# yu45020/Text_Segmentation_Image_Inpainting

Hardware: NVIDIA H100
Metric: PartialConv UNet 512x512 images/sec (fwd+bwd) (higher is better)
Workload: dtype bf16

## Files before the change

### text_segmentation_image_inpainting_b200/csrc/conv_stem.cu

```cuda
#include <string.h>

#include <algorithm>

#include "pcb_common.cuh"

namespace {

constexpr int S2D_C = 32;
constexpr int SK = 4;

size_t rup256(size_t v) { return (v + 255) / 256 * 256; }
size_t s2d_bytes(const pcb_conv *c) { return rup256(static_cast<size_t>(c->n) * (c->h / 2) * (c->w / 2) * S2D_C * sizeof(bf16)); }
size_t dwsub_bytes(const pcb_conv *c) { return rup256(sizeof(float) * c->cout * SK * SK * S2D_C); }

}

StemPlan pcb_stem_plan(const pcb_conv *c) {
    StemPlan K;
    memset(&K, 0, sizeof(K));
    if (c->dtype != PCB_BF16 || c->groups != 1 || c->nparts != 1 || c->kh != 7 || c->kw != 7 || c->stride != 2 || c->pad_h != 3 || c->pad_w != 3 ||
        c->dil != 1) return K;
    const pcb_part &p = c->parts[0];
    if (p.x_up || p.c > 8 || p.x_cstride != 8 || (p.mask && p.mask_up != 0) || ((c->h | c->w) & 1)) return K;
    if (p.x && (reinterpret_cast<uintptr_t>(p.x) & 15)) return K;
    if (c->ho != c->h / 2 || c->wo != c->w / 2 || c->cout < 32 || (c->cout & 7)) return K;
    pcb_conv &S = K.sub;
    S.n = c->n; S.h = c->h / 2; S.w = c->w / 2; S.cin = S2D_C; S.cout = c->cout; S.kh = S.kw = SK; S.stride = 1; S.pad_h = S.pad_w = 2; S.dil = 1;
    S.groups = 1; S.ho = S.h; S.wo = S.w; S.dtype = PCB_BF16; S.no_guard = c->no_guard; S.nparts = 1;
    S.parts[0].x = nullptr; S.parts[0].mask = nullptr; S.parts[0].c = S2D_C; S.parts[0].x_cstride = S2D_C;
    if (!pcb_tc_eligible(&S)) return K;
    size_t de;
    pcb_tc_weight_layout(&S, &K.sub_fe, &de);
    K.sub_fe = (K.sub_fe + 63) / 64 * 64;
    K.fwd_extra = K.sub_fe + 2 * static_cast<size_t>(c->cout) * SK * SK * S2D_C;
    K.workspace = s2d_bytes(c) + dwsub_bytes(c) + pcb_tc_workspace(&S);
    K.ok = true;
    return K;
// ... 8 lines not shown
        const int a = static_cast<int>(i & 1);
        const long long cell = i >> 1;
        const int sx = static_cast<int>(cell % ws);
        const long long t = cell / ws;
        const int sy = static_cast<int>(t % hs), img = static_cast<int>(t / hs);
        const long long q = (static_cast<long long>(img) * h + 2 * sy + a) * w + 2 * sx;
        uint4 v0 = __ldg(reinterpret_cast<const uint4 *>(x + q * 8)), v1 = __ldg(reinterpret_cast<const uint4 *>(x + q * 8 + 8));
        if (mask) {
            if (mask[q] == 0) v0 = make_uint4(0u, 0u, 0u, 0u);
            if (mask[q + 1] == 0) v1 = make_uint4(0u, 0u, 0u, 0u);
        }
        uint4 *dst = reinterpret_cast<uint4 *>(xs + cell * S2D_C + a * 16);
        dst[0] = v0; dst[1] = v1;
    }
}

__global__ void stem_weight_kernel(const float *__restrict__ w, float *__restrict__ wsub, int cout, int cin) {
    const int i = blockIdx.x * blockDim.x + threadIdx.x;
    if (i >= cout * SK * SK * S2D_C) return;
    const int k = i % S2D_C, jb = (i / S2D_C) % SK, ja = (i / (S2D_C * SK)) % SK, co = i / (S2D_C * SK * SK);
    const int ch = k & 7, b = (k >> 3) & 1, a = k >> 4;
    const int ty = 2 * ja + a - 1, tx = 2 * jb + b - 1;
    wsub[i] = (ty >= 0 && ty < 7 && tx >= 0 && tx < 7 && ch < cin) ? w[((static_cast<long long>(co) * 7 + ty) * 7 + tx) * cin + ch] : 0.f;
}

__global__ void stem_dw_gather_kernel(const float *__restrict__ dwsub, float *__restrict__ dw, int cout, int cin) {
    const int i = blockIdx.x * blockDim.x + threadIdx.x;
    if (i >= cout * 49 * cin) return;
    const int ch = i % cin, tx = (i / cin) % 7, ty = (i / (cin * 7)) % 7, co = i / (cin * 49);
    const int ja = (ty + 1) >> 1, a = (ty + 1) & 1, jb = (tx + 1) >> 1, b = (tx + 1) & 1;
    dw[i] += dwsub[((static_cast<long long>(co) * SK + ja) * SK + jb) * S2D_C + (a * 2 + b) * 8 + ch];
}

int run_s2d(const pcb_conv *c, bf16 *xs, cudaStream_t st) {
    const pcb_part &p = c->parts[0];
    PCB_CHECK(p.x != nullptr, "space-to-depth stem: null x");
    const long long total = static_cast<long long>(c->n) * (c->h / 2) * (c->w / 2) * 2;
    const int grid = static_cast<int>(std::max<long long>(1, std::min<long long>((total + 255) / 256, 16ll * pcb_num_sms())));
    s2d_kernel<<<grid, 256, 0, st>>>(static_cast<const bf16 *>(p.x), p.mask, xs, c->n, c->h, c->w);
    PCB_LAUNCH_CHECK();
    return 0;
}

}

int pcb_stem_weight_prepare(const pcb_conv *c, const StemPlan &K, const float *w_master, void *w_fwd_extra, bool zero_padding, cudaStream_t st) {
    PCB_CHECK(K.ok && w_fwd_extra, "space-to-depth stem: weight prepare on a layer that does not take this path");
    float *wsub = reinterpret_cast<float *>(static_cast<bf16 *>(w_fwd_extra) + K.sub_fe);
    const int total = c->cout * SK * SK * S2D_C;
    stem_weight_kernel<<<(total + 255) / 256, 256, 0, st>>>(w_master, wsub, c->cout, c->cin);
    PCB_LAUNCH_CHECK();
    return pcb_tc_weight_prepare(&K.sub, wsub, w_fwd_extra, nullptr, zero_padding, st);
}

int pcb_stem_forward(const pcb_conv *c, const StemPlan &K, const void *w_fwd_extra, const float *bias, void *y, int y_cstride,
                     const float *msum, void *workspace, double *bn_sums, const pcb_ep *ep, cudaStream_t st) {
    PCB_CHECK(K.ok && workspace, "space-to-depth stem forward: wrong layer / no workspace");
    uint8_t *ws = static_cast<uint8_t *>(workspace);
    bf16 *xs = reinterpret_cast<bf16 *>(ws);
    if (int rc = run_s2d(c, xs, st)) return rc;
    pcb_conv sub = K.sub;
    sub.parts[0].x = xs;
    uint64_t *sub_ws = reinterpret_cast<uint64_t *>(ws + s2d_bytes(c) + dwsub_bytes(c));
    if (int rc = pcb_tc_forward_mask_pass(&sub, sub_ws, st)) return rc;
    return pcb_tc_forward_ws(&sub, w_fwd_extra, bias, y, y_cstride, msum, sub_ws, true, bn_sums, ep, st);
}

int pcb_stem_wgrad(const pcb_conv *c, const StemPlan &K, const void *dc, int dc_cstride, float *dw, void *workspace, bool zero_dw,
                   cudaStream_t st) {
    PCB_CHECK(K.ok && workspace, "space-to-depth stem wgrad: wrong layer / no workspace");
    if (zero_dw) PCB_CUDA(cudaMemsetAsync(dw, 0, sizeof(float) * c->cout * 49 * c->cin, st));
    uint8_t *ws = static_cast<uint8_t *>(workspace);
    bf16 *xs = reinterpret_cast<bf16 *>(ws);
    float *dwsub = reinterpret_cast<float *>(ws + s2d_bytes(c));
    void *sub_ws = ws + s2d_bytes(c) + dwsub_bytes(c);
    if (int rc = run_s2d(c, xs, st)) return rc;
    pcb_conv sub = K.sub;
    sub.parts[0].x = xs;
    if (int rc = pcb_tc_wgrad(&sub, dc, dc_cstride, dwsub, sub_ws, true, st)) return rc;
    const int total = c->cout * 49 * c->cin;
    stem_dw_gather_kernel<<<(total + 255) / 256, 256, 0, st>>>(dwsub, dw, c->cout, c->cin);
    PCB_LAUNCH_CHECK();
    return 0;
}
```

### text_segmentation_image_inpainting_b200/csrc/conv_tc.cu

```cuda
#include <cuda.h>
#include <stdlib.h>
#include <string.h>

#include <algorithm>

#include "pcb_common.cuh"
#include "pcb_ptx.cuh"

namespace {

constexpr int BLOCK_M = 128;
constexpr int BLOCK_K = 64;
constexpr int A_STAGE_BYTES = BLOCK_M * 128;
constexpr int NUM_PRODUCER_THREADS = 128;
constexpr int TC_MAX_PARTS = 2;
constexpr int MMA_WARPS = 8;
constexpr int MMA_THREADS = MMA_WARPS * 32;
constexpr int acc_pitch(int block_n) { return block_n + 4; }
constexpr int acc_stage_bytes(int block_n) { return BLOCK_M * acc_pitch(block_n) * 4; }

inline int rup(int v, int m) { return (v + m - 1) / m * m; }

struct TcPart {
    const bf16 *x;
// ... 1781 lines not shown
#pragma unroll
        for (int i = 0; i < 4; ++i) {
            const int ci = ci0 + ty + 8 * i;
            if (co < P.cout && ci < P.cin) {
                int p = 0;
                while (p + 1 < P.nparts && ci >= P.choff[p] + P.c[p]) ++p;
                const int kpos = P.koff[p] + (ci - P.choff[p]);
                w_dg[static_cast<long long>(kpos) * P.kd + static_cast<long long>(tap) * P.cout64 + co] = __float2bfloat16_rn(tile[tx][ty + 8 * i]);
            }
        }
    }
}

__global__ void tc_weight_prepare_kernel(const float *__restrict__ wm, const WPrepParams P, bf16 *__restrict__ w_fwd, bf16 *__restrict__ w_dg) {
    const long long total = static_cast<long long>(P.cout) * P.taps * P.cin;
    for (long long i = blockIdx.x * static_cast<long long>(blockDim.x) + threadIdx.x; i < total; i += static_cast<long long>(gridDim.x) * blockDim.x) {
        const int ci = static_cast<int>(i % P.cin);
        const long long t = i / P.cin;
        const int tap = static_cast<int>(t % P.taps), co = static_cast<int>(t / P.taps);
        const bf16 v = __float2bfloat16_rn(wm[i]);
        if (P.rowpack) {
            const int tr = tap / P.kw, tc = tap - tr * P.kw;
            w_fwd[static_cast<long long>(co) * P.kf + tr * 64 + tc * 8 + ci] = v;
        } else {
            int p = 0;
            while (p + 1 < P.nparts && ci >= P.choff[p] + P.c[p]) ++p;
            const int kpos = P.koff[p] + (ci - P.choff[p]);
            w_fwd[static_cast<long long>(co) * P.kf + static_cast<long long>(tap) * P.ktap + kpos] = v;
            if (w_dg) w_dg[static_cast<long long>(kpos) * P.kd + static_cast<long long>(tap) * P.cout64 + co] = v;
        }
    }
}

typedef CUresult (*EncodeTiledFn)(CUtensorMap *, CUtensorMapDataType, cuuint32_t, void *, const cuuint64_t *,
                                  const cuuint64_t *, const cuuint32_t *, const cuuint32_t *, CUtensorMapInterleave,
                                  CUtensorMapSwizzle, CUtensorMapL2promotion, CUtensorMapFloatOOBfill);

EncodeTiledFn get_encode_fn() {
    static EncodeTiledFn fn = nullptr;
    if (!fn) {
        void *p = nullptr;
        cudaDriverEntryPointQueryResult qres;
        if (cudaGetDriverEntryPoint("cuTensorMapEncodeTiled", &p, cudaEnableDefault, &qres) == cudaSuccess &&
            qres == cudaDriverEntryPointSuccess)
            fn = reinterpret_cast<EncodeTiledFn>(p);
    }
    return fn;
}

int make_tmap_2d(CUtensorMap *tm, const void *base, long long rows, long long cols, long long pitch_elems, int box_rows) {
    EncodeTiledFn enc = get_encode_fn();
    PCB_CHECK(enc != nullptr, "cuTensorMapEncodeTiled not available from the driver");
    cuuint64_t dims[2] = {static_cast<cuuint64_t>(cols), static_cast<cuuint64_t>(rows)};
    cuuint64_t strides[1] = {static_cast<cuuint64_t>(pitch_elems) * 2};
    cuuint32_t box[2] = {64, static_cast<cuuint32_t>(box_rows)};
    cuuint32_t estr[2] = {1, 1};
    CUresult r = enc(tm, CU_TENSOR_MAP_DATA_TYPE_BFLOAT16, 2, const_cast<void *>(base), dims, strides, box, estr,
                     CU_TENSOR_MAP_INTERLEAVE_NONE, CU_TENSOR_MAP_SWIZZLE_128B, CU_TENSOR_MAP_L2_PROMOTION_L2_256B,
                     CU_TENSOR_MAP_FLOAT_OOB_FILL_NONE);
    PCB_CHECK(r == CUDA_SUCCESS, "cuTensorMapEncodeTiled failed (%d) rows=%lld cols=%lld pitch=%lld box_rows=%d base=%p", (int)r,
              rows, cols, pitch_elems, box_rows, base);
    return 0;
}

int make_tmap_nhwc(CUtensorMap *tm, const void *base, int channels, int w, int h, int n, long long cstride, int bx, int by, int bn, int es) {
    EncodeTiledFn enc = get_encode_fn();
    PCB_CHECK(enc != nullptr, "cuTensorMapEncodeTiled not available from the driver");
    cuuint64_t dims[4] = {static_cast<cuuint64_t>(channels), static_cast<cuuint64_t>(w), static_cast<cuuint64_t>(h), static_cast<cuuint64_t>(n)};
    cuuint64_t strides[3] = {static_cast<cuuint64_t>(cstride) * 2, static_cast<cuuint64_t>(w) * cstride * 2, static_cast<cuuint64_t>(h) * w * cstride * 2};
    cuuint32_t box[4] = {64, static_cast<cuuint32_t>(bx * es), static_cast<cuuint32_t>(by * es), static_cast<cuuint32_t>(bn)};
    cuuint32_t estr[4] = {1, static_cast<cuuint32_t>(es), static_cast<cuuint32_t>(es), 1};
    CUresult r = enc(tm, CU_TENSOR_MAP_DATA_TYPE_BFLOAT16, 4, const_cast<void *>(base), dims, strides, box, estr,
                     CU_TENSOR_MAP_INTERLEAVE_NONE, CU_TENSOR_MAP_SWIZZLE_128B, CU_TENSOR_MAP_L2_PROMOTION_L2_256B,
                     CU_TENSOR_MAP_FLOAT_OOB_FILL_NONE);
    PCB_CHECK(r == CUDA_SUCCESS, "cuTensorMapEncodeTiled(4D) failed (%d) c=%d w=%d h=%d n=%d cstride=%lld box=%d,%d,%d es=%d base=%p", (int)r,
              channels, w, h, n, cstride, bx, by, bn, es, base);
    return 0;
}

int *abort_flag_ptr() {
    static int *flag[PCB_MAX_DEVICES] = {};
    const int dev = pcb_cur_device();
    if (!flag[dev]) {
        if (cudaMalloc(&flag[dev], sizeof(int)) != cudaSuccess) { flag[dev] = nullptr; return nullptr; }
        cudaMemset(flag[dev], 0, sizeof(int));
    }
    return flag[dev];
}

bool is_rowpack(const pcb_conv *c) { return c->nparts == 1 && c->cin <= 8 && c->kw <= 8 && c->parts[0].x_up == 0; }

bool common_ok(const pcb_conv *c) {
    if (c->dtype != PCB_BF16 || c->groups != 1 || c->kh * c->kw > 64) return false;
    if (c->stride & (c->stride - 1)) return false;
    const long long lim = (1ll << 31) - 1;
    if (static_cast<long long>(c->n) * c->ho * c->wo * rup(c->cout, 64) > lim) return false;
    if (c->nparts < 1 || c->nparts > TC_MAX_PARTS) return false;
    for (int p = 0; p < c->nparts; ++p) {
        const pcb_part &pt = c->parts[p];
        if (pt.x_cstride % 8 != 0 || pt.x_cstride < rup(pt.c, 8)) return false;
        if (static_cast<long long>(c->n) * (c->h >> pt.x_up) * (c->w >> pt.x_up) * pt.x_cstride > lim) return false;
        if (pt.x && (reinterpret_cast<uintptr_t>(pt.x) & 15)) return false;
    }
    if (is_rowpack(c)) return c->cout >= 16;
    return c->cin >= 32 || c->cout >= 32;
}

struct Layout {
    int rowpack, ktap, cout64, rows_f, bn_f;
    long long kf, kd;
    int koff[TC_MAX_PARTS], kext[TC_MAX_PARTS];
};

Layout layout_of(const pcb_conv *c) {
    Layout L;
    memset(&L, 0, sizeof(L));
    L.rowpack = is_rowpack(c);
    const int taps = c->kh * c->kw;
    if (L.rowpack) {
        L.ktap = 64; L.koff[0] = 0; L.kext[0] = 64;
        L.kf = static_cast<long long>(c->kh) * 64;
// ... 605 lines not shown
    const DirPlan &F = T.fwd;
    PCB_CHECK(T.m_out < (1ll << 31), "problem too large");
    PCB_CHECK(y_cstride % 8 == 0 && y_cstride >= c->cout, "tensor-core forward: y channel stride must be a multiple of 8 and >= cout");
    PCB_CHECK(bn_sums == nullptr || T.fuses_epilogue, "fused BatchNorm statistics requested from a kernel that does not produce them");
    PCB_CHECK(ep == nullptr || T.fuses_epilogue, "fused BatchNorm + activation requested from a kernel that does not apply it");
    if (!mask_pass_done && T.fwd_tapmask)
        if (int rc = launch_tapmask(c, tapmask, st)) return rc;
    const bf16 *wf = static_cast<const bf16 *>(w_fwd);
    if (F.route == ROUTE_STEM) return pcb_stem_forward(c, T.stem, wf + T.extra_fwd_off, bias, y, y_cstride, msum, tapmask, bn_sums, ep, st);
    if (F.route == ROUTE_K2R) return pcb_k2r_forward(c, T.k2r, smallco_layout(L), w_fwd, wf + T.extra_fwd_off, bias, y, y_cstride, msum, tapmask, st);
    if (F.route == ROUTE_SMALLCO) return pcb_smallco_forward(c, smallco_layout(L), w_fwd, bias, y, y_cstride, msum, st);
    TcParams P;
    base_params(P, c, L);
    P.m_total = static_cast<int>(T.m_out);
    fill_parts(c, L, P.parts, tapmask, T.m_out);
    P.bias = bias; P.msum = msum; P.y = static_cast<bf16 *>(y); P.y_cstride = y_cstride; P.abort_flag = flag;
    P.bn_sums = bn_sums; P.bn_c = c->cout;
    set_ep(P, ep);
    P.ncols = L.rows_f;
    CUtensorMap tm;
    if (int rc = make_tmap_2d(&tm, w_fwd, L.rows_f, L.kf, L.kf, F.bn)) return rc;
    if (F.route == ROUTE_TMA) {
        P.box_w = F.box_w; P.box_h = F.box_h; P.box_n = F.box_n;
        CUtensorMap ta[TC_MAX_PARTS];
        if (int rc = a_operand_maps(c, T, tapmask, F.box_w + (F.halo ? (c->kw - 1) * c->dil : 0), F.box_h, F.box_n, ta, &P.use_fix, st)) return rc;
        P.ncols = (c->cout <= 32) ? 32 : L.rows_f;
        P.wk_base = 0; P.wk_col = L.ktap; P.wk_row = c->kw * L.ktap;
        return launch_tma<0>(P, tm, ta[0], ta[1], F.bn, F.halo, st);
    }
    P.hg = F.hg;
    return launch_tc<0>(P, tm, F.bn, st);
}

bool pcb_tc_dgrad_fuses_relu(const pcb_conv *c) { return tc_plan(c).dg_fuses_relu; }

int pcb_tc_dgrad(const pcb_conv *c, const void *dc, int dc_cstride, const void *w_dgrad, void *const *dx, const int *dx_cstride,
                 cudaStream_t st, const void *relu_x, int relu_cstride) {
    const TcPlan T = tc_plan(c);
    const Layout &L = T.L;
    const DirPlan &D = T.dg;
    PCB_CHECK(D.route != ROUTE_NONE, "data gradient of a row-packed (cin <= 8) tensor-core layer: set force_generic and pass KRSC weights");
    PCB_CHECK(w_dgrad != nullptr && (reinterpret_cast<uintptr_t>(dc) & 15) == 0, "pcb_pconv_backward_data: w_dgrad required / dc misaligned");
    PCB_CHECK(relu_x == nullptr || (T.dg_fuses_relu && relu_cstride % 8 == 0 && relu_cstride >= rup(c->cin, 8) &&
                                    (reinterpret_cast<uintptr_t>(relu_x) & 15) == 0),
              "tensor-core dgrad: the ReLU backward is fused only on the TMA-fed stride-1 kernel (16-byte aligned input, channel stride %% 8 == 0)");
    int *flag = abort_flag_ptr();
    PCB_CHECK(flag != nullptr, "cudaMalloc(abort flag) failed");
    PCB_CHECK(T.m_in < (1ll << 31), "problem too large");
    PCB_CHECK(dc_cstride % 8 == 0 && dc_cstride >= rup(c->cout, 8), "tensor-core dgrad: dc channel stride must be a multiple of 8");
    const bf16 *wd = static_cast<const bf16 *>(w_dgrad);
    if (D.route == ROUTE_K2R) return pcb_k2r_dgrad(c, T.k2r, smallco_layout(L), dc, dc_cstride, w_dgrad, wd + T.extra_dg_off, dx, dx_cstride, st);
    if (D.route == ROUTE_SMALLCO) return pcb_smallco_dgrad(c, smallco_layout(L), dc, dc_cstride, w_dgrad, dx, dx_cstride, st);
    const SpPlan &SPL = T.sp;
    void *dx_local[TC_MAX_PARTS] = {nullptr, nullptr};
    for (int p = 0; p < c->nparts && p < TC_MAX_PARTS; ++p) dx_local[p] = dx[p];
    if (SPL.ok) {
        if (dx[SPL.pu] != nullptr)
            if (int rc = sp_dgrad_up(c, SPL, L, dc, dc_cstride, wd + T.sp_off, dx[SPL.pu], dx_cstride[SPL.pu], flag, st)) return rc;
        dx_local[SPL.pu] = nullptr;
        if (SPL.ps < 0 || dx[SPL.ps] == nullptr) return 0;
    }
    dx = dx_local;
    TcParams P;
    base_params(P, c, L);
    P.m_total = static_cast<int>(T.m_in);
    fill_parts(c, L, P.parts, nullptr, 0);
// ... 148 lines not shown
```

### text_segmentation_image_inpainting_b200/csrc/pcb_common.cuh

```cuda
#pragma once
#include <cuda_bf16.h>
#include <cuda_runtime.h>
#include <stdint.h>
#include <stdio.h>

#include "../../include/pconv_b200.h"

int pcb_set_error(const char *fmt, ...);
void pcb_count_launch(int n = 1);

#define PCB_CHECK(cond, ...)                       \
    do {                                           \
        if (!(cond)) return pcb_set_error(__VA_ARGS__); \
    } while (0)

#define PCB_CUDA(expr)                                                                           \
    do {                                                                                         \
        cudaError_t _e = (expr);                                                                 \
        if (_e != cudaSuccess)                                                                   \
            return pcb_set_error("%s:%d: %s -> %s", __FILE__, __LINE__, #expr, cudaGetErrorString(_e)); \
    } while (0)

#define PCB_LAUNCH_CHECK()                                                                        \
    do {                                                                                         \
        cudaError_t _e = cudaGetLastError();                                                     \
        if (_e != cudaSuccess)                                                                   \
            return pcb_set_error("%s:%d: kernel launch -> %s", __FILE__, __LINE__, cudaGetErrorString(_e)); \
        pcb_count_launch();                                                                      \
    } while (0)

constexpr int PCB_MAX_DEVICES = 64;

static inline int pcb_cur_device() {
// ... 69 lines not shown
    }
};
template <> struct Vec8<float> {
    static __device__ __forceinline__ void load(const float *p, float (&v)[8]) {
        float4 a = reinterpret_cast<const float4 *>(p)[0], b = reinterpret_cast<const float4 *>(p)[1];
        v[0] = a.x; v[1] = a.y; v[2] = a.z; v[3] = a.w; v[4] = b.x; v[5] = b.y; v[6] = b.z; v[7] = b.w;
    }
    static __device__ __forceinline__ void store(float *p, const float (&v)[8]) {
        reinterpret_cast<float4 *>(p)[0] = make_float4(v[0], v[1], v[2], v[3]);
        reinterpret_cast<float4 *>(p)[1] = make_float4(v[4], v[5], v[6], v[7]);
    }
};

__device__ __forceinline__ float warp_sum(float v) {
#pragma unroll
    for (int o = 16; o > 0; o >>= 1) v += __shfl_xor_sync(0xffffffffu, v, o);
    return v;
}

struct pcb_ep { const float *scale, *shift; int act; float slope; };

int pcb_generic_forward(const pcb_conv *c, const void *w, const float *bias, void *y, int y_cstride, const float *msum, cudaStream_t st);
int pcb_generic_dgrad(const pcb_conv *c, const void *dc, int dc_cstride, const void *w_krsc, void *const *dx, const int *dx_cstride,
                      cudaStream_t st);
int pcb_generic_wgrad(const pcb_conv *c, const void *dc, int dc_cstride, float *dw, bool zero_dw, cudaStream_t st);
int pcb_mask_sums(const pcb_conv *c, float *msum, uint8_t *newmask, cudaStream_t st);
bool pcb_tc_eligible(const pcb_conv *c);
size_t pcb_tc_workspace(const pcb_conv *c);
void pcb_tc_weight_layout(const pcb_conv *c, size_t *fwd_elems, size_t *dgrad_elems);
int pcb_tc_weight_prepare(const pcb_conv *c, const float *w_master, void *w_fwd, void *w_dgrad, bool zero_padding, cudaStream_t st);
int pcb_tc_forward_mask_pass(const pcb_conv *c, uint64_t *tapmask, cudaStream_t st);
int pcb_tc_forward_ws(const pcb_conv *c, const void *w_fwd, const float *bias, void *y, int y_cstride, const float *msum,
                      uint64_t *tapmask, bool mask_pass_done, double *bn_sums, const pcb_ep *ep, cudaStream_t st);
bool pcb_tc_fuses_epilogue(const pcb_conv *c);
bool pcb_tc_subpixel(const pcb_conv *c);
int pcb_tc_dgrad(const pcb_conv *c, const void *dc, int dc_cstride, const void *w_dgrad, void *const *dx, const int *dx_cstride,
                 cudaStream_t st, const void *relu_x = nullptr, int relu_cstride = 0);
bool pcb_tc_dgrad_fuses_relu(const pcb_conv *c);
int pcb_tc_wgrad(const pcb_conv *c, const void *dc, int dc_cstride, float *dw, void *workspace, bool zero_dw, cudaStream_t st);
int pcb_tc_read_abort_flag(int *value);
struct pcb_smallco_layout { int ktap, koff[2], cout64; long long kf, kd; };
bool pcb_smallco_eligible(const pcb_conv *c);
int pcb_smallco_forward(const pcb_conv *c, const pcb_smallco_layout &L, const void *w_fwd, const float *bias, void *y, int y_cstride, const float *msum,
                        cudaStream_t st);
int pcb_smallco_dgrad(const pcb_conv *c, const pcb_smallco_layout &L, const void *dc, int dc_cstride, const void *w_dgrad, void *const *dx, const int *dx_cstride,
                      cudaStream_t st);
int pcb_smallco_wgrad(const pcb_conv *c, const pcb_smallco_layout &L, const void *dc, int dc_cstride, float *dw, bool zero_dw, cudaStream_t st);
struct K2rPlan {
    bool ok;
    int pu, ps;
    int cu, cs, choff_u, choff_s;
    pcb_conv sub;
    size_t sub_fe, sub_de;
    size_t fwd_extra, dg_extra;
    size_t workspace;
};
K2rPlan pcb_k2r_plan(const pcb_conv *c);
int pcb_k2r_weight_prepare(const pcb_conv *c, const K2rPlan &K, const float *w_master, void *w_fwd_extra, void *w_dg_extra, bool zero_padding,
                           cudaStream_t st);
int pcb_k2r_forward(const pcb_conv *c, const K2rPlan &K, const pcb_smallco_layout &L, const void *w_fwd, const void *w_fwd_extra, const float *bias,
                    void *y, int y_cstride, const float *msum, void *workspace, cudaStream_t st);
int pcb_k2r_dgrad(const pcb_conv *c, const K2rPlan &K, const pcb_smallco_layout &L, const void *dc, int dc_cstride, const void *w_dgrad,
                  const void *w_dg_extra, void *const *dx, const int *dx_cstride, cudaStream_t st);
int pcb_k2r_wgrad(const pcb_conv *c, const K2rPlan &K, const void *dc, int dc_cstride, float *dw, void *workspace, bool zero_dw, cudaStream_t st);
struct StemPlan {
    bool ok;
    pcb_conv sub;
    size_t sub_fe;
    size_t fwd_extra;
    size_t workspace;
};
StemPlan pcb_stem_plan(const pcb_conv *c);
int pcb_stem_weight_prepare(const pcb_conv *c, const StemPlan &K, const float *w_master, void *w_fwd_extra, bool zero_padding, cudaStream_t st);
// ... 12 lines not shown
```

### text_segmentation_image_inpainting_b200/csrc/pcb_ptx.cuh

```cuda
#pragma once
#include <cuda.h>
#include <cuda_runtime.h>
#include <stdint.h>

namespace ptx {

__device__ __forceinline__ uint32_t smem_u32(const void *p) { return static_cast<uint32_t>(__cvta_generic_to_shared(p)); }

__device__ __forceinline__ bool elect_one() {
    uint32_t pred = 0;
    asm volatile(
        "{\n\t.reg .pred P;\n\telect.sync _|P, 0xffffffff;\n\tselp.b32 %0, 1, 0, P;\n\t}" : "=r"(pred));
    return pred != 0;
}

__device__ __forceinline__ void mbar_init(uint32_t bar, uint32_t count) {
    asm volatile("mbarrier.init.shared::cta.b64 [%0], %1;" ::"r"(bar), "r"(count) : "memory");
}
__device__ __forceinline__ void fence_mbar_init() { asm volatile("fence.mbarrier_init.release.cluster;" ::: "memory"); }
__device__ __forceinline__ void mbar_arrive(uint32_t bar) {
    asm volatile("mbarrier.arrive.shared::cta.b64 _, [%0];" ::"r"(bar) : "memory");
}
__device__ __forceinline__ void mbar_arrive_expect_tx(uint32_t bar, uint32_t bytes) {
    asm volatile("mbarrier.arrive.expect_tx.shared::cta.b64 _, [%0], %1;" ::"r"(bar), "r"(bytes) : "memory");
// ... 78 lines not shown
        : "l"(a_desc), "l"(b_desc), "n"(TA), "n"(TB));
}
template <int TA, int TB> __device__ __forceinline__ void wgmma_m64n128(float (&d)[64], uint64_t a_desc, uint64_t b_desc) {
    asm volatile(
        "{\n\t"
        "wgmma.mma_async.sync.aligned.m64n128k16.f32.bf16.bf16 "
        "{%0, %1, %2, %3, %4, %5, %6, %7, %8, %9, %10, %11, %12, %13, %14, %15, %16, %17, %18, %19, %20, %21, %22, %23, %24, %25, %26, %27, %28, %29, %30, %31, %32, %33, %34, %35, %36, %37, %38, %39, %40, %41, %42, %43, %44, %45, %46, %47, %48, %49, %50, %51, %52, %53, %54, %55, %56, %57, %58, %59, %60, %61, %62, %63}, %64, %65, 1, 1, 1, %66, %67;\n\t"
        "}"
        : "+f"(d[0]), "+f"(d[1]), "+f"(d[2]), "+f"(d[3]), "+f"(d[4]), "+f"(d[5]), "+f"(d[6]), "+f"(d[7]), "+f"(d[8]), "+f"(d[9]), "+f"(d[10]), "+f"(d[11]), "+f"(d[12]), "+f"(d[13]), "+f"(d[14]), "+f"(d[15]), "+f"(d[16]), "+f"(d[17]), "+f"(d[18]), "+f"(d[19]), "+f"(d[20]), "+f"(d[21]), "+f"(d[22]), "+f"(d[23]), "+f"(d[24]), "+f"(d[25]), "+f"(d[26]), "+f"(d[27]), "+f"(d[28]), "+f"(d[29]), "+f"(d[30]), "+f"(d[31]), "+f"(d[32]), "+f"(d[33]), "+f"(d[34]), "+f"(d[35]), "+f"(d[36]), "+f"(d[37]), "+f"(d[38]), "+f"(d[39]), "+f"(d[40]), "+f"(d[41]), "+f"(d[42]), "+f"(d[43]), "+f"(d[44]), "+f"(d[45]), "+f"(d[46]), "+f"(d[47]), "+f"(d[48]), "+f"(d[49]), "+f"(d[50]), "+f"(d[51]), "+f"(d[52]), "+f"(d[53]), "+f"(d[54]), "+f"(d[55]), "+f"(d[56]), "+f"(d[57]), "+f"(d[58]), "+f"(d[59]), "+f"(d[60]), "+f"(d[61]), "+f"(d[62]), "+f"(d[63])
        : "l"(a_desc), "l"(b_desc), "n"(TA), "n"(TB));
}
template <int N, int TA, int TB> __device__ __forceinline__ void wgmma_bf16(float (&d)[N / 2], uint64_t a_desc, uint64_t b_desc) {
    if constexpr (N == 32) wgmma_m64n32<TA, TB>(d, a_desc, b_desc);
    else if constexpr (N == 64) wgmma_m64n64<TA, TB>(d, a_desc, b_desc);
    else if constexpr (N == 128) wgmma_m64n128<TA, TB>(d, a_desc, b_desc);
    else {
        static_assert(N == 256 && TB == 0, "wgmma tile width");
        wgmma_m64n128<TA, TB>(*reinterpret_cast<float (*)[64]>(&d[0]), a_desc, b_desc);
        wgmma_m64n128<TA, TB>(*reinterpret_cast<float (*)[64]>(&d[64]), a_desc, b_desc + (16384 >> 4));
    }
}
template <int N> __device__ __forceinline__ void setmaxnreg_inc() { asm volatile("setmaxnreg.inc.sync.aligned.u32 %0;" ::"n"(N)); }
template <int N> __device__ __forceinline__ void setmaxnreg_dec() { asm volatile("setmaxnreg.dec.sync.aligned.u32 %0;" ::"n"(N)); }
__device__ __forceinline__ void named_sync(int id, int threads) { asm volatile("bar.sync %0, %1;" ::"r"(id), "r"(threads) : "memory"); }

__host__ __device__ __forceinline__ uint64_t make_smem_desc(uint32_t smem_addr, uint32_t lbo_bytes, uint32_t sbo_bytes) {
    uint64_t d = 0;
    d |= static_cast<uint64_t>((smem_addr >> 4) & 0x3FFFu);
    d |= static_cast<uint64_t>((lbo_bytes >> 4) & 0x3FFFu) << 16;
    d |= static_cast<uint64_t>((sbo_bytes >> 4) & 0x3FFFu) << 32;
    d |= 1ull << 62;
    return d;
}
__host__ __device__ __forceinline__ uint64_t make_smem_desc_noswizzle(uint32_t smem_addr, uint32_t lbo_bytes, uint32_t sbo_bytes) {
    uint64_t d = 0;
    d |= static_cast<uint64_t>((smem_addr >> 4) & 0x3FFFu);
    d |= static_cast<uint64_t>((lbo_bytes >> 4) & 0x3FFFu) << 16;
    d |= static_cast<uint64_t>((sbo_bytes >> 4) & 0x3FFFu) << 32;
    return d;
}

}
```

Measured before the change: 974.7.

## Add dedicated TMA-based stem forward and wgrad kernels for space-to-depth conv

Adds a specialized warp-specialized forward kernel for the 4x4 space-to-depth stem that keeps all 16 weight taps resident in shared memory and streams one image-row strip per tap row via 4D TMA, skipping the separate mask pass. Adds a dedicated wgrad kernel that loads shifted input strips and output-gradient tiles via TMA and accumulates into dwsub with atomics across split-K CTAs. Both target the first layer at full resolution, where the generic implicit-GEMM path wastes bandwidth and per-tap gathers. They add large shared-memory footprints and atomic contention, and only take effect for specific shapes (cout 64, width multiples of 128 or 64).

```diff
diff --git a/text_segmentation_image_inpainting_b200/csrc/conv_stem.cu b/text_segmentation_image_inpainting_b200/csrc/conv_stem.cu
--- a/text_segmentation_image_inpainting_b200/csrc/conv_stem.cu
+++ b/text_segmentation_image_inpainting_b200/csrc/conv_stem.cu
@@ -3,6 +3,7 @@
 #include <algorithm>
 
 #include "pcb_common.cuh"
+#include "pcb_ptx.cuh"
 
 namespace {
 
@@ -77,6 +78,138 @@
     dw[i] += dwsub[((static_cast<long long>(co) * SK + ja) * SK + jb) * S2D_C + (a * 2 + b) * 8 + ch];
 }
 
+constexpr int SW_THREADS = 2 * 128 + 32;
+constexpr int SW_CELLS = 64 + SK - 1;
+constexpr uint32_t SW_A_BYTES = (SW_CELLS * 64 + 511) & ~511u;
+constexpr uint32_t SW_B_BYTES = 64 * 128;
+constexpr uint32_t SW_STAGE = SK * SW_A_BYTES + SW_B_BYTES;
+constexpr uint32_t SW_TX = SK * SW_CELLS * 64 + SW_B_BYTES;
+constexpr int SW_RING = 6;
+constexpr size_t SW_SMEM = 1024 + SW_RING * SW_STAGE + 16 * SW_RING;
+static_assert(SW_STAGE % 1024 == 0 && (SK * SW_A_BYTES) % 1024 == 0, "stem wgrad stage alignment");
+
+struct StemWgParams {
+    int ho, wo, cout, kb_per_cta, total_kb;
+    float *dwsub;
+    int *abort_flag;
+};
+
+template <int BLOCK_N>
+__global__ void __launch_bounds__(SW_THREADS, 1)
+stem_wgrad_kernel(const __grid_constant__ StemWgParams P, const __grid_constant__ CUtensorMap tmap_dc, const __grid_constant__ CUtensorMap tmap_xs) {
+    extern __shared__ uint8_t smem_raw[];
+    const uint32_t smem_base = (ptx::smem_u32(smem_raw) + 1023u) & ~1023u;
+    const uint32_t sBar = smem_base + SW_RING * SW_STAGE;
+    const uint32_t bar_full = sBar, bar_empty = sBar + 8 * SW_RING;
+    const int warp = __shfl_sync(0xffffffffu, threadIdx.x >> 5, 0), lane = threadIdx.x & 31;
+    const int n0 = blockIdx.y * 64;
+    const int kb_begin = blockIdx.x * P.kb_per_cta;
+    const int num_kb = max(0, min(P.total_kb, kb_begin + P.kb_per_cta) - kb_begin);
+
+    if (threadIdx.x == 0) {
+        for (int s = 0; s < SW_RING; ++s) {
+            ptx::mbar_init(bar_full + 8 * s, 1);
+            ptx::mbar_init(bar_empty + 8 * s, 2);
+        }
+        ptx::fence_mbar_init();
+    }
+    if (warp == 8 && lane == 0) { ptx::prefetch_tmap(&tmap_dc); ptx::prefetch_tmap(&tmap_xs); }
+    __syncthreads();
+    if (warp < 8) {
+        const int g = warp >> 2;
+        const bool leader = (threadIdx.x & 127) == 0;
+        const uint64_t desc_a0 = ptx::make_smem_desc_sw64(smem_base + 2 * g * SW_A_BYTES, 64, 512);
+        const uint64_t desc_b0 = ptx::make_smem_desc(smem_base + SK * SW_A_BYTES, 8192, 1024);
+        float acc[4][BLOCK_N / 2];
+#pragma unroll
+        for (int q = 0; q < 4; ++q)
+#pragma unroll
+            for (int i = 0; i < BLOCK_N / 2; ++i) acc[q][i] = 0.f;
+        int s = 0, held = -1;
+        uint32_t ph = 0;
+        bool dead = false;
+        for (int it = 0; it < num_kb; ++it) {
+            if (!__all_sync(0xffffffffu, ptx::mbar_wait(bar_full + 8 * s, ph, P.abort_flag, 231))) { dead = true; break; }
+            const uint64_t st16 = static_cast<uint64_t>(s * (SW_STAGE >> 4));
+            ptx::wgmma_fence();
+#pragma unroll
+            for (int q = 0; q < 4; ++q) {
+                const uint64_t da = desc_a0 + st16 + (((q >> 1) * SW_A_BYTES + (q & 1) * 128) >> 4);
+#pragma unroll
+                for (int k = 0; k < 4; ++k)
+                    ptx::wgmma_bf16<BLOCK_N, 1, 1>(acc[q], da + 64 * k, desc_b0 + st16 + 128 * k);
+            }
+            ptx::wgmma_commit();
+            ptx::wgmma_wait<1>();
+            if (held >= 0 && leader) ptx::mbar_arrive(bar_empty + 8 * held);
+            held = s;
+            if (++s == SW_RING) { s = 0; ph ^= 1; }
+        }
+        ptx::wgmma_wait<0>();
+#pragma unroll
+        for (int q = 0; q < 4; ++q) ptx::wgmma_fence_regs(acc[q]);
+        if (held >= 0 && leader) ptx::mbar_arrive(bar_empty + 8 * held);
+        if (!dead && num_kb > 0) {
+#pragma unroll
+            for (int q = 0; q < 4; ++q) {
+                const int jy = 2 * g + (q >> 1);
+#pragma unroll
+                for (int i = 0; i < BLOCK_N / 2; ++i) {
+                    const int row = 16 * (warp & 3) + (lane >> 2) + 8 * ((i >> 1) & 1);
+                    const int jx = 2 * (q & 1) + (row >> 5);
+                    const int co = n0 + 8 * (i >> 2) + 2 * (lane & 3) + (i & 1);
+                    if (co < P.cout) atomicAdd(P.dwsub + ((co * SK + jy) * SK + jx) * S2D_C + (row & 31), acc[q][i]);
+                }
+            }
+        }
+    } else if (lane == 0) {
+        const int plane = P.ho * P.wo;
+        int s = 0;
+        uint32_t ph = 1;
+        for (int it = 0; it < num_kb; ++it) {
+            const int m0 = (kb_begin + it) * 64;
+            const int img = m0 / plane, rem = m0 - img * plane;
+            const int oy = rem / P.wo, ox = rem - oy * P.wo;
+            if (!ptx::mbar_wait(bar_empty + 8 * s, ph, P.abort_flag, 232)) break;
+            const uint32_t full = bar_full + 8 * s, dst = smem_base + s * SW_STAGE;
+            ptx::mbar_arrive_expect_tx(full, SW_TX);
+#pragma unroll
+            for (int jy = 0; jy < SK; ++jy) ptx::tma_load_4d(dst + jy * SW_A_BYTES, &tmap_xs, 0, ox - 2, oy + jy - 2, img, full);
+            ptx::tma_load_2d(dst + SK * SW_A_BYTES, &tmap_dc, n0, m0, full);
+            if (++s == SW_RING) { s = 0; ph ^= 1; }
+        }
+    }
+}
+
+template <int BLOCK_N>
+int launch_stem_wgrad(const pcb_conv *S, const bf16 *xs, const void *dc, int dc_cstride, float *dwsub, cudaStream_t st) {
+    int *flag = abort_flag_ptr();
+    PCB_CHECK(flag != nullptr, "cudaMalloc(abort flag) failed");
+    const long long m_total = static_cast<long long>(S->n) * S->ho * S->wo;
+    PCB_CHECK(m_total < (1ll << 31), "space-to-depth stem wgrad: problem too large");
+    CUtensorMap tdc, txs;
+    if (int rc = make_tmap_2d(&tdc, dc, m_total, S->cout, dc_cstride, 64)) return rc;
+    EncodeTiledFn enc = get_encode_fn();
+    PCB_CHECK(enc != nullptr, "cuTensorMapEncodeTiled not available from the driver");
+    const cuuint64_t dims[4] = {S2D_C, static_cast<cuuint64_t>(S->w), static_cast<cuuint64_t>(S->h), static_cast<cuuint64_t>(S->n)};
+    const cuuint64_t strides[3] = {S2D_C * 2, static_cast<cuuint64_t>(S->w) * S2D_C * 2, static_cast<cuuint64_t>(S->h) * S->w * S2D_C * 2};
+    const cuuint32_t box[4] = {S2D_C, SW_CELLS, 1, 1}, estr[4] = {1, 1, 1, 1};
+    CUresult r = enc(&txs, CU_TENSOR_MAP_DATA_TYPE_BFLOAT16, 4, const_cast<bf16 *>(xs), dims, strides, box, estr, CU_TENSOR_MAP_INTERLEAVE_NONE,
+                     CU_TENSOR_MAP_SWIZZLE_64B, CU_TENSOR_MAP_L2_PROMOTION_L2_256B, CU_TENSOR_MAP_FLOAT_OOB_FILL_NONE);
+    PCB_CHECK(r == CUDA_SUCCESS, "cuTensorMapEncodeTiled(space-to-depth) failed (%d)", (int)r);
+    StemWgParams P;
+    P.ho = S->ho; P.wo = S->wo; P.cout = S->cout; P.dwsub = dwsub; P.abort_flag = flag;
+    P.total_kb = static_cast<int>(m_total / 64);
+    const int co_tiles = (S->cout + 63) / 64;
+    const int ctas = std::max(1, std::min(P.total_kb, pcb_num_sms() / co_tiles));
+    P.kb_per_cta = (P.total_kb + ctas - 1) / ctas;
+    auto kern = stem_wgrad_kernel<BLOCK_N>;
+    PCB_SMEM_OPT_IN(kern, SW_SMEM);
+    kern<<<dim3((P.total_kb + P.kb_per_cta - 1) / P.kb_per_cta, co_tiles), SW_THREADS, SW_SMEM, st>>>(P, tdc, txs);
+    PCB_LAUNCH_CHECK();
+    return 0;
+}
+
 int run_s2d(const pcb_conv *c, bf16 *xs, cudaStream_t st) {
     const pcb_part &p = c->parts[0];
     PCB_CHECK(p.x != nullptr, "space-to-depth stem: null x");
@@ -106,6 +239,7 @@
     if (int rc = run_s2d(c, xs, st)) return rc;
     pcb_conv sub = K.sub;
     sub.parts[0].x = xs;
+    if (sub.cout == 64 && sub.wo % 128 == 0) return pcb_tc_stem_forward(&sub, w_fwd_extra, bias, y, y_cstride, msum, bn_sums, ep, st);
     uint64_t *sub_ws = reinterpret_cast<uint64_t *>(ws + s2d_bytes(c) + dwsub_bytes(c));
     if (int rc = pcb_tc_forward_mask_pass(&sub, sub_ws, st)) return rc;
     return pcb_tc_forward_ws(&sub, w_fwd_extra, bias, y, y_cstride, msum, sub_ws, true, bn_sums, ep, st);
@@ -122,7 +256,14 @@
     if (int rc = run_s2d(c, xs, st)) return rc;
     pcb_conv sub = K.sub;
     sub.parts[0].x = xs;
-    if (int rc = pcb_tc_wgrad(&sub, dc, dc_cstride, dwsub, sub_ws, true, st)) return rc;
+    if (sub.wo % 64 == 0) {
+        PCB_CHECK(dc_cstride % 8 == 0 && dc_cstride >= c->cout, "space-to-depth stem wgrad: dc channel stride must be a multiple of 8");
+        PCB_CUDA(cudaMemsetAsync(dwsub, 0, sizeof(float) * c->cout * SK * SK * S2D_C, st));
+        if (int rc = c->cout <= 32 ? launch_stem_wgrad<32>(&sub, xs, dc, dc_cstride, dwsub, st) : launch_stem_wgrad<64>(&sub, xs, dc, dc_cstride, dwsub, st))
+            return rc;
+    } else if (int rc = pcb_tc_wgrad(&sub, dc, dc_cstride, dwsub, sub_ws, true, st)) {
+        return rc;
+    }
     const int total = c->cout * 49 * c->cin;
     stem_dw_gather_kernel<<<(total + 255) / 256, 256, 0, st>>>(dwsub, dw, c->cout, c->cin);
     PCB_LAUNCH_CHECK();
diff --git a/text_segmentation_image_inpainting_b200/csrc/conv_tc.cu b/text_segmentation_image_inpainting_b200/csrc/conv_tc.cu
--- a/text_segmentation_image_inpainting_b200/csrc/conv_tc.cu
+++ b/text_segmentation_image_inpainting_b200/csrc/conv_tc.cu
@@ -1837,9 +1837,115 @@
     }
 }
 
-typedef CUresult (*EncodeTiledFn)(CUtensorMap *, CUtensorMapDataType, cuuint32_t, void *, const cuuint64_t *,
-                                  const cuuint64_t *, const cuuint32_t *, const cuuint32_t *, CUtensorMapInterleave,
-                                  CUtensorMapSwizzle, CUtensorMapL2promotion, CUtensorMapFloatOOBfill);
+constexpr int STEM_RING = 12;
+constexpr int STEM_CELLS = BLOCK_M + 3;
+constexpr uint32_t STEM_A_BYTES = (STEM_CELLS * 64 + 511) & ~511u;
+constexpr uint32_t STEM_W_BYTES = 16 * 64 * 64;
+constexpr uint32_t STEM_BAR_BYTES = 16 * STEM_RING + 32;
+constexpr size_t STEM_SMEM = 1024 + STEM_W_BYTES + STEM_RING * STEM_A_BYTES + STEM_BAR_BYTES + EPI_STAT_SMEM_BYTES + bf16_stage_bytes(64);
+static_assert(STEM_SMEM <= 227 * 1024 && (STEM_A_BYTES % 512) == 0, "stem forward shared memory");
+
+__global__ void __maxnreg__(TMA_REGS)
+stem_fwd_kernel(const __grid_constant__ TcParams P, const __grid_constant__ CUtensorMap tmap_w, const __grid_constant__ CUtensorMap tmap_a) {
+    constexpr int BLOCK_N = 64;
+    extern __shared__ uint8_t smem_raw[];
+    const uint32_t smem_base = align1024(ptx::smem_u32(smem_raw));
+    const uint32_t sW = smem_base, sA = smem_base + STEM_W_BYTES;
+    const uint32_t sBar = sA + STEM_RING * STEM_A_BYTES;
+    const uint32_t bar_full = sBar, bar_empty = sBar + 8 * STEM_RING;
+    const uint32_t w_full = sBar + 16 * STEM_RING, acc_full = w_full + 8, acc_empty = w_full + 16;
+    const uint32_t s_stat_addr = sBar + STEM_BAR_BYTES;
+    const uint32_t s_acc = s_stat_addr + EPI_STAT_SMEM_BYTES;
+    uint8_t *smem_gen = smem_raw + (smem_base - ptx::smem_u32(smem_raw));
+
+    const int warp = __shfl_sync(0xffffffffu, threadIdx.x >> 5, 0), lane = threadIdx.x & 31;
+    const int num_tiles = (P.m_total + BLOCK_M - 1) / BLOCK_M;
+    const int tile0 = static_cast<int>(blockIdx.x), tstep = static_cast<int>(gridDim.x);
+
+    if (threadIdx.x == 0) {
+        for (int s = 0; s < STEM_RING; ++s) { ptx::mbar_init(bar_full + 8 * s, 1); ptx::mbar_init(bar_empty + 8 * s, 2); }
+        ptx::mbar_init(w_full, 1);
+        ptx::mbar_init(acc_full, MMA_WARPS); ptx::mbar_init(acc_empty, EPI_WARPS);
+        ptx::fence_mbar_init();
+    }
+    if (warp == 8 && lane == 0) { ptx::prefetch_tmap(&tmap_w); ptx::prefetch_tmap(&tmap_a); }
+    __syncthreads();
+
+    bf16 *acc_stage = reinterpret_cast<bf16 *>(smem_gen + (s_acc - smem_base));
+    if (warp < MMA_WARPS) {
+        ptx::setmaxnreg_inc<TMA_CONSUMER_REGS>();
+        const int e = warp, g = warp >> 2;
+        const bool leader = (threadIdx.x & 127) == 0;
+        const uint64_t desc_a0 = ptx::make_smem_desc_sw64(sA + g * 64 * 64, 16, 512);
+        const uint64_t desc_w0 = ptx::make_smem_desc_sw64(sW, 16, 512);
+        constexpr uint32_t stage16 = STEM_A_BYTES >> 4;
+        int s = 0;
+        uint32_t ph = 0, aph = 1;
+        bool dead = !__all_sync(0xffffffffu, ptx::mbar_wait(w_full, 0, P.abort_flag, 131));
+        for (int tile = tile0; tile < num_tiles && !dead; tile += tstep) {
+            const ConsRows cr = cons_rows<0>(P, tile * BLOCK_M, e, lane);
+            float acc[BLOCK_N / 2];
+            zero_acc(acc);
+            int held = -1;
+            for (int tr = 0; tr < 4; ++tr) {
+                if (!__all_sync(0xffffffffu, ptx::mbar_wait(bar_full + 8 * s, ph, P.abort_flag, 132))) { dead = true; break; }
+                const uint64_t da = desc_a0 + static_cast<uint64_t>(s * stage16);
+                ptx::wgmma_fence();
+#pragma unroll
+                for (int tc = 0; tc < 4; ++tc)
+#pragma unroll
+                    for (int k = 0; k < 2; ++k)
+                        ptx::wgmma_bf16<BLOCK_N, 0, 0>(acc, da + 4 * tc + 2 * k, desc_w0 + ((tr * 4 + tc) * 4096 >> 4) + 2 * k);
+                ptx::wgmma_commit();
+                ptx::wgmma_wait<1>();
+                if (held >= 0 && leader) ptx::mbar_arrive(bar_empty + 8 * held);
+                held = s;
+                if (++s == STEM_RING) { s = 0; ph ^= 1; }
+            }
+            ptx::wgmma_wait<0>();
+            ptx::wgmma_fence_regs(acc);
+            if (held >= 0 && leader) ptx::mbar_arrive(bar_empty + 8 * held);
+            if (dead) break;
+            if (!tma_stage_tile<BLOCK_N, 0>(P, acc, acc_stage, acc_full, acc_empty, aph, e, lane, 0, cr, 133)) break;
+        }
+    } else {
+        ptx::setmaxnreg_dec<TMA_SUPPORT_REGS>();
+        if (warp >= EPI_WARP0) {
+            const int w = warp - EPI_WARP0;
+            float *s_stat = P.bn_sums != nullptr ? reinterpret_cast<float *>(smem_gen + (s_stat_addr - smem_base)) + w * EPI_STAT_SLICE : nullptr;
+            int stat_n0 = -1;
+            auto origin = [&](int tile, int &m0, int &n0) { m0 = tile * BLOCK_M; n0 = 0; };
+            tma_epilogue_warps<BLOCK_N, 0>(P, tile0, tstep, num_tiles, origin, acc_stage, acc_full, acc_empty, s_stat, stat_n0, w, lane, 134);
+            ptx::named_sync(1, EPI_WARPS * 32);
+            if (s_stat != nullptr && stat_n0 >= 0) tc_stats_final<BLOCK_N>(P, s_stat - w * EPI_STAT_SLICE, w, lane, stat_n0);
+        } else if (warp == 8) {
+            if (ptx::elect_one()) {
+                ptx::mbar_arrive_expect_tx(w_full, STEM_W_BYTES);
+                for (int tap = 0; tap < 16; ++tap) ptx::tma_load_2d(sW + tap * 4096, &tmap_w, tap * P.ktap, 0, w_full);
+            }
+            __syncwarp();
+            const int plane = P.ho * P.wo;
+            int s = 0;
+            uint32_t ph = 1;
+            bool dead = false;
+            for (int tile = tile0; tile < num_tiles && !dead; tile += tstep) {
+                const int m0 = tile * BLOCK_M, img = m0 / plane, rem = m0 - img * plane;
+                const int oy = rem / P.wo, ox = rem - oy * P.wo;
+                for (int tr = 0; tr < 4; ++tr) {
+                    if (!__all_sync(0xffffffffu, ptx::mbar_wait(bar_empty + 8 * s, ph, P.abort_flag, 135))) { dead = true; break; }
+                    if (ptx::elect_one()) {
+                        ptx::mbar_arrive_expect_tx(bar_full + 8 * s, STEM_CELLS * 64);
+                        ptx::tma_load_4d(sA + s * STEM_A_BYTES, &tmap_a, 0, ox - P.pad_w, oy - P.pad_h + tr, img, bar_full + 8 * s);
+                    }
+                    __syncwarp();
+                    if (++s == STEM_RING) { s = 0; ph ^= 1; }
+                }
+            }
+        }
+    }
+}
+
+}
 
 EncodeTiledFn get_encode_fn() {
     static EncodeTiledFn fn = nullptr;
@@ -1892,6 +1998,8 @@
     }
     return flag[dev];
 }
+
+namespace {
 
 bool is_rowpack(const pcb_conv *c) { return c->nparts == 1 && c->cin <= 8 && c->kw <= 8 && c->parts[0].x_up == 0; }
 
@@ -2563,6 +2671,43 @@
     return launch_tc<0>(P, tm, F.bn, st);
 }
 
+int pcb_tc_stem_forward(const pcb_conv *c, const void *w_fwd, const float *bias, void *y, int y_cstride, const float *msum, double *bn_sums,
+                        const pcb_ep *ep, cudaStream_t st) {
+    int *flag = abort_flag_ptr();
+    PCB_CHECK(flag != nullptr, "cudaMalloc(abort flag) failed");
+    const TcPlan T = tc_plan(c);
+    const Layout &L = T.L;
+    PCB_CHECK(T.fwd.route == ROUTE_TMA && c->cout == 64 && c->cin == 32 && c->kh == 4 && c->kw == 4 && c->wo % BLOCK_M == 0 && L.ktap == 64 &&
+              T.fuses_epilogue && T.m_out < (1ll << 31), "stem forward kernel: not the space-to-depth stem's 4x4 problem");
+    PCB_CHECK(y_cstride % 8 == 0 && y_cstride >= c->cout, "tensor-core forward: y channel stride must be a multiple of 8 and >= cout");
+    TcParams P;
+    base_params(P, c, L);
+    P.m_total = static_cast<int>(T.m_out);
+    P.bias = bias; P.msum = msum; P.y = static_cast<bf16 *>(y); P.y_cstride = y_cstride; P.abort_flag = flag;
+    P.bn_sums = bn_sums; P.bn_c = c->cout;
+    set_ep(P, ep);
+    P.ncols = 64;
+    EncodeTiledFn enc = get_encode_fn();
+    PCB_CHECK(enc != nullptr, "cuTensorMapEncodeTiled not available from the driver");
+    CUtensorMap tw, ta;
+    const cuuint64_t wdims[2] = {static_cast<cuuint64_t>(L.kf), static_cast<cuuint64_t>(L.rows_f)}, wstr[1] = {static_cast<cuuint64_t>(L.kf) * 2};
+    const cuuint32_t wbox[2] = {32, 64}, westr[2] = {1, 1};
+    CUresult r = enc(&tw, CU_TENSOR_MAP_DATA_TYPE_BFLOAT16, 2, const_cast<void *>(w_fwd), wdims, wstr, wbox, westr, CU_TENSOR_MAP_INTERLEAVE_NONE,
+                     CU_TENSOR_MAP_SWIZZLE_64B, CU_TENSOR_MAP_L2_PROMOTION_L2_256B, CU_TENSOR_MAP_FLOAT_OOB_FILL_NONE);
+    PCB_CHECK(r == CUDA_SUCCESS, "cuTensorMapEncodeTiled(stem weights) failed (%d)", (int)r);
+    const cuuint64_t adims[4] = {32, static_cast<cuuint64_t>(c->w), static_cast<cuuint64_t>(c->h), static_cast<cuuint64_t>(c->n)};
+    const cuuint64_t astr[3] = {64, static_cast<cuuint64_t>(c->w) * 64, static_cast<cuuint64_t>(c->h) * c->w * 64};
+    const cuuint32_t abox[4] = {32, STEM_CELLS, 1, 1}, aestr[4] = {1, 1, 1, 1};
+    r = enc(&ta, CU_TENSOR_MAP_DATA_TYPE_BFLOAT16, 4, const_cast<void *>(static_cast<const void *>(c->parts[0].x)), adims, astr, abox, aestr, CU_TENSOR_MAP_INTERLEAVE_NONE,
+            CU_TENSOR_MAP_SWIZZLE_64B, CU_TENSOR_MAP_L2_PROMOTION_L2_256B, CU_TENSOR_MAP_FLOAT_OOB_FILL_NONE);
+    PCB_CHECK(r == CUDA_SUCCESS, "cuTensorMapEncodeTiled(space-to-depth image) failed (%d)", (int)r);
+    PCB_SMEM_OPT_IN(stem_fwd_kernel, STEM_SMEM);
+    const int grid = std::min(static_cast<int>(T.m_out / BLOCK_M), pcb_num_sms());
+    stem_fwd_kernel<<<grid, TMA_THREADS, STEM_SMEM, st>>>(P, tw, ta);
+    PCB_LAUNCH_CHECK();
+    return 0;
+}
+
 bool pcb_tc_dgrad_fuses_relu(const pcb_conv *c) { return tc_plan(c).dg_fuses_relu; }
 
 int pcb_tc_dgrad(const pcb_conv *c, const void *dc, int dc_cstride, const void *w_dgrad, void *const *dx, const int *dx_cstride,
diff --git a/text_segmentation_image_inpainting_b200/csrc/pcb_common.cuh b/text_segmentation_image_inpainting_b200/csrc/pcb_common.cuh
--- a/text_segmentation_image_inpainting_b200/csrc/pcb_common.cuh
+++ b/text_segmentation_image_inpainting_b200/csrc/pcb_common.cuh
@@ -1,4 +1,5 @@
 #pragma once
+#include <cuda.h>
 #include <cuda_bf16.h>
 #include <cuda_runtime.h>
 #include <stdint.h>
@@ -134,6 +135,8 @@
 int pcb_tc_forward_mask_pass(const pcb_conv *c, uint64_t *tapmask, cudaStream_t st);
 int pcb_tc_forward_ws(const pcb_conv *c, const void *w_fwd, const float *bias, void *y, int y_cstride, const float *msum,
                       uint64_t *tapmask, bool mask_pass_done, double *bn_sums, const pcb_ep *ep, cudaStream_t st);
+int pcb_tc_stem_forward(const pcb_conv *c, const void *w_fwd, const float *bias, void *y, int y_cstride, const float *msum, double *bn_sums,
+                        const pcb_ep *ep, cudaStream_t st);
 bool pcb_tc_fuses_epilogue(const pcb_conv *c);
 bool pcb_tc_subpixel(const pcb_conv *c);
 int pcb_tc_dgrad(const pcb_conv *c, const void *dc, int dc_cstride, const void *w_dgrad, void *const *dx, const int *dx_cstride,
@@ -141,6 +144,12 @@
 bool pcb_tc_dgrad_fuses_relu(const pcb_conv *c);
 int pcb_tc_wgrad(const pcb_conv *c, const void *dc, int dc_cstride, float *dw, void *workspace, bool zero_dw, cudaStream_t st);
 int pcb_tc_read_abort_flag(int *value);
+typedef CUresult (*EncodeTiledFn)(CUtensorMap *, CUtensorMapDataType, cuuint32_t, void *, const cuuint64_t *,
+                                  const cuuint64_t *, const cuuint32_t *, const cuuint32_t *, CUtensorMapInterleave,
+                                  CUtensorMapSwizzle, CUtensorMapL2promotion, CUtensorMapFloatOOBfill);
+EncodeTiledFn get_encode_fn();
+int make_tmap_2d(CUtensorMap *tm, const void *base, long long rows, long long cols, long long pitch_elems, int box_rows);
+int *abort_flag_ptr();
 struct pcb_smallco_layout { int ktap, koff[2], cout64; long long kf, kd; };
 bool pcb_smallco_eligible(const pcb_conv *c);
 int pcb_smallco_forward(const pcb_conv *c, const pcb_smallco_layout &L, const void *w_fwd, const float *bias, void *y, int y_cstride, const float *msum,
diff --git a/text_segmentation_image_inpainting_b200/csrc/pcb_ptx.cuh b/text_segmentation_image_inpainting_b200/csrc/pcb_ptx.cuh
--- a/text_segmentation_image_inpainting_b200/csrc/pcb_ptx.cuh
+++ b/text_segmentation_image_inpainting_b200/csrc/pcb_ptx.cuh
@@ -134,6 +134,9 @@
     d |= 1ull << 62;
     return d;
 }
+__host__ __device__ __forceinline__ uint64_t make_smem_desc_sw64(uint32_t smem_addr, uint32_t lbo_bytes, uint32_t sbo_bytes) {
+    return (make_smem_desc(smem_addr, lbo_bytes, sbo_bytes) & ~(3ull << 62)) | (2ull << 62);
+}
 __host__ __device__ __forceinline__ uint64_t make_smem_desc_noswizzle(uint32_t smem_addr, uint32_t lbo_bytes, uint32_t sbo_bytes) {
     uint64_t d = 0;
     d |= static_cast<uint64_t>((smem_addr >> 4) & 0x3FFFu);
```

Result: faster. 1017 (median of 6 runs) (+4.3%).
